# Danderson123/Amira

Hardware: AMD Instinct MI355X
Metric: gene-mers/s to corrected GeneMerGraph (higher is better)
Workload: dtype int32; 1 GPU; synthetic 1M reads x 60 genes, k=5, 20k-gene vocab: build + error-correction sweep (build, filter(3,1), correct, build, clip(5), correct, build); reads_per_gpu=1000000, genes_per_read=60, k=5, vocab=20000, gene_mers_per_gpu=56000000, final_nodes=472478, final_edges=1054844, multi_gpu=n/a

## Files before the change

### amira_amd/csrc/amg_api.hip

```cpp
#include <cstdarg>

#include "amg_device.h"

thread_local std::string g_amg_err;

int amg_fail(int code, const char* fmt, ...) {
  char buf[1024];
  va_list ap;
  va_start(ap, fmt);
  vsnprintf(buf, sizeof(buf), fmt, ap);
  va_end(ap);
  g_amg_err = buf;
  return code;
}

extern "C" const char* amg_last_error(void) { return g_amg_err.c_str(); }

void stages_reset(amg_ctx* c) {
  for (auto& s : c->stages) {
    (void)hipEventDestroy(s.a);
    (void)hipEventDestroy(s.b);
  }
  c->stages.clear();
}
// ... 122 lines not shown
  if (device < 0 || device >= n) return amg_fail(AMG_E_ARG, "device %d out of range [0,%d)", device, n);
  HIPCHK(hipSetDevice(device));
  amg_ctx* c = new amg_ctx();
  c->device = device;
  e = hipStreamCreateWithFlags(&c->stream, hipStreamNonBlocking);
  if (e != hipSuccess) {
    delete c;
    return amg_fail(AMG_E_HIP, "hipStreamCreate: %s", hipGetErrorString(e));
  }
  int r = c->status.ensure(ST_WORDS * sizeof(unsigned long long));
  if (r != AMG_OK) {
    delete c;
    return r;
  }
  const char* t = getenv("AMG_TIMING");
  c->timing = !(t && t[0] == '0');
  *out = c;
  return AMG_OK;
}

extern "C" int amg_destroy(amg_ctx* c) {
  if (!c) return AMG_OK;
  (void)hipSetDevice(c->device);
  (void)hipStreamSynchronize(c->stream);
  stages_reset(c);
  dist_release(c);
  bubbles_release(c);
  sketch_release(c);
  pop_release(c);
  DevBuf* all[] = {&c->tokens,    &c->read_off,  &c->gene_start, &c->gene_end,  &c->read_len,
                   &c->node_tab,  &c->edge_tab,  &c->tok_slot,   &c->tok_node,  &c->tok_dir, &c->tok_pair,
                   &c->node_tokens, &c->node_cov, &c->node_first, &c->node_comp, &c->node_alive,
                   &c->edge_src,  &c->edge_tgt,  &c->edge_sdir,  &c->edge_tdir, &c->edge_cov,
                   &c->edge_alive, &c->adj_off,  &c->adj_edge,   &c->read_fix, &c->ladj, &c->ladj_rows, &c->ladj_pos, &c->ladj_keys, &c->hub_bits, &c->pair_key, &c->pair_first, &c->pair_cnt, &c->match_read, &c->match_pos, &c->match_off, &c->match_wave,  &c->c_tokens_buf,
                   &c->c_read_off, &c->c_orig,   &c->c_changed,  &c->c_gstart,  &c->c_gend,
                   &c->c_read_len, &c->status,   &c->sort_tmp, &c->scan_state,   &c->s0, &c->s1, &c->s2, &c->s3,
                   &c->s4, &c->s5, &c->cnt_state, &c->cnt_list, &c->bnd_bits, &c->nw_rec, &c->gap_rec, &c->gm_mask, &c->gm_tab, &c->gm_res, &c->gm_list, &c->gm_q, &c->gm_pool, &c->gm_gene, &c->gm_fail, &c->gm_ctr, &c->routes_dev, &c->nw_big, &c->x_first, &c->x_slot, &c->x_final, &c->x_efirst, &c->x_eslot, &c->x_ecnt, &c->x_ncnt, &c->x_ftag, &c->f_ctrs, &c->x_first_all, &c->pos_off, &c->c_pos_off, &c->pos1_s, &c->pos1_e,
                   &c->c_src, &c->rd_src, &c->alt_tok_node, &c->alt_tok_dir, &c->alt_ntok, &c->alt_ncov, &c->alt_nfirst,
                   &c->alt_nalive, &c->alt_pkey, &c->alt_pfirst, &c->alt_pcnt};
  for (DevBuf* b : all) b->release();
  if (c->mail_host) (void)hipHostFree(c->mail_host);
  (void)hipStreamDestroy(c->stream);
  delete c;
  return AMG_OK;
}

extern "C" int amg_sync(amg_ctx* c) {
  if (!c) return amg_fail(AMG_E_ARG, "null ctx");
  HIPCHK(hipStreamSynchronize(c->stream));
  return AMG_OK;
}

extern "C" void* amg_stream(amg_ctx* c) { return c ? (void*)c->stream : nullptr; }

static int copy_in(amg_ctx* c, DevBuf& dst, const void* src, size_t bytes, int on_device) {
  if (on_device == 2) {
    dst.borrow(src, bytes);
    return AMG_OK;
  }
  AMGCHK(dst.ensure(bytes + 64));
  if (bytes)
    HIPCHK(hipMemcpyAsync(dst.p, src, bytes, on_device ? hipMemcpyDeviceToDevice : hipMemcpyHostToDevice,
                          c->stream));
  return AMG_OK;
}

extern "C" int amg_set_reads(amg_ctx* c, const int32_t* tokens, const int64_t* read_offsets,
// ... 322 lines not shown
```

### amira_amd/csrc/amg_correct.h

```cpp
#pragma once
#include "amg_device.h"

enum { RC_SKIP = 0, RC_COPY = 1, RC_DROP = 2, RC_TRIM = 3, RC_GAPPED = 4, RC_KEEP_ORIG = 5 };

struct CorrArgs {
  const int* tokens;
  const long long* read_off;
  const int* tok_node;
  const signed char* tok_dir;
  const unsigned char* read_fix;
  const long long* p0s;
  const long long* p0e;
  const long long* p1s;
  const long long* p1e;
  long long n0;
  const long long* pos_off;
  const long long* read_len;
  long long n_reads;
  int k, flip, have_pos;
  unsigned int* gflag;
  unsigned long long* max_bound;
  unsigned long long* lmask;
  unsigned long long* n_runs;
  unsigned char* cls;
  unsigned char* cls_final;
  int* r_start;
  int* r_end;
  unsigned int* bound;
  const long long* tmp_off;
  unsigned int* new_len;
  int* tmp_tok;
};

__device__ __forceinline__ void pos_base(const CorrArgs& a, long long off, const long long*& gs, const long long*& ge) {
  if (off < a.n0) {
    gs = a.p0s + off;
    ge = a.p0e + off;
  } else {
    gs = a.p1s + (off - a.n0);
    ge = a.p1e + (off - a.n0);
  }
}

// ... 136 lines not shown
  long long* o_off;
  int* o_orig;
  unsigned char* o_changed;
  long long* o_src;
  const long long* pos_new;
  long long* o_posoff;
  long long* o_rl;
  long long out_reads, out_tokens;
  unsigned long long* dead_kept;
};

struct CorrSwitches {
  bool gap_memo;
  bool gap_dfs_wave;
  bool fast_gapped;
  bool lean_gapped;
  int fast_nw;
  int nw_shortcuts;
  const char* node_bound;
  bool routes;
  const char* gap_pool;
  const char* memo_spill;
};

struct CorrScratch {
  size_t per_read = 0;
  unsigned char *cls = nullptr, *final_cls = nullptr;
  int *r_start = nullptr, *r_end = nullptr;
  long long *nw_size = nullptr, *nw_off = nullptr;
  unsigned int *bound = nullptr, *new_len = nullptr, *flag = nullptr;
  long long *tmp_off = nullptr, *new_idx = nullptr, *new_off = nullptr;
  int* tmp_tok = nullptr;
  long long *plen = nullptr, *poffs = nullptr, *pos_new = nullptr;
  unsigned long long *max_bound = nullptr, *n_general = nullptr;
  unsigned long long* n_runs = nullptr;
  unsigned long long* dead_kept = nullptr;
  bool count_alive = false;
  DevBuf* glist = nullptr;
  DevBuf* cand = nullptr;
  DevBuf* pool = nullptr;
  DevBuf* need_slow = nullptr;
};

struct CorrCounts {
  long long tmp_total = 0, n_gapped = 0, total_runs = 0;
  unsigned long long max_bound = 0;
  bool carry = false;
  long long out_reads = 0, out_tokens = 0, big_total = 0, pos_total = 0;
  unsigned long long n_general = 0;
  long long n_queries = 0;
  int pool_retries = 0;
  bool lean_ran = false, fast_ran = false, memo = false;
};

static void fill_pos_args(amg_ctx* c, CorrArgs& a) {
  a.p0s = c->have_pos ? c->gene_start.as<long long>() : nullptr;
  a.p0e = c->have_pos ? c->gene_end.as<long long>() : nullptr;
  a.p1s = c->pos1_s.as<long long>();
  a.p1e = c->pos1_e.as<long long>();
  a.n0 = c->pos_n0;
  a.pos_off = (c->have_pos && !c->pos_identity) ? c->pos_off.as<long long>() : nullptr;
}

int corr_gapped(amg_ctx* c, const CorrSwitches& sw, const CorrScratch& S, const CorrArgs& a, CorrCounts& n);
int corr_nw_sizes(amg_ctx* c, const CorrSwitches& sw, const CorrScratch& S, const CorrArgs& a, long long n_gapped,
                  FetchList& shape);
int corr_grow_pos_pools(amg_ctx* c, const CorrCounts& n);
int corr_positions(amg_ctx* c, const CorrSwitches& sw, const CorrScratch& S, const CorrArgs& a, const CorrCounts& n,
// ... 17 lines not shown
```

### amira_amd/csrc/amg_correct.hip

```cpp
#include "amg_correct.h"

__global__ __launch_bounds__(256) void k_count_alive(const unsigned char* __restrict__ alive, long long n,
                                                     unsigned long long* out) {
  __shared__ unsigned int s_part[4];
  unsigned int c = 0;
  for (long long i = ((long long)blockIdx.x * blockDim.x + threadIdx.x) * 4; i < n; i += (long long)gridDim.x * blockDim.x * 4) {
    if (i + 4 <= n) {
      const unsigned int w = *reinterpret_cast<const unsigned int*>(alive + i);
      c += __popc(w & 0x01010101u);
    } else {
      for (long long j = i; j < n; ++j) c += alive[j] ? 1u : 0u;
    }
  }
  for (int d = 32; d > 0; d >>= 1) c += (unsigned int)__shfl_xor((int)c, d, 64);
  if ((threadIdx.x & 63) == 0) s_part[threadIdx.x >> 6] = c;
  __syncthreads();
  if (threadIdx.x == 0 && (s_part[0] | s_part[1] | s_part[2] | s_part[3]))
    atomicAdd(out, (unsigned long long)s_part[0] + s_part[1] + s_part[2] + s_part[3]);
}

__global__ __launch_bounds__(256) void k_corr_classify(CorrArgs a) {
  const long long rbase = ((long long)blockIdx.x * 4 + (threadIdx.x >> 6)) * CLS_READS;
  if (rbase >= a.n_reads) return;
  const int lane = threadIdx.x & 63;
  const long long r = rbase + lane;
  const bool have = r < a.n_reads;
  const long long t0 = have ? a.read_off[r] : 0;
  const long long n = have ? (a.read_off[r + 1] - t0) - a.k + 1 : 0;
  const bool look = have && n > 0 && a.read_fix[r] != 0;
  unsigned long long lv = 0;
  unsigned long long todo = __ballot(look && n <= 64);
  while (todo) {
    int who[4];
    long long tj[4];
    int nj[4], v[4];
#pragma unroll
    for (int q = 0; q < 4; ++q) {
      who[q] = todo ? __ffsll((long long)todo) - 1 : -1;
      if (todo) todo &= todo - 1ull;
      tj[q] = who[q] >= 0 ? bcast_i64(t0, who[q]) : 0;
      nj[q] = who[q] >= 0 ? __builtin_amdgcn_readlane((int)n, who[q]) : 0;
    }
#pragma unroll
    for (int q = 0; q < 4; ++q) v[q] = lane < nj[q] ? a.tok_node[tj[q] + lane] : -1;
#pragma unroll
    for (int q = 0; q < 4; ++q) {
      const unsigned long long m = __ballot(v[q] >= 0);
      if (lane == who[q]) lv = m;
    }
  }
  long long first = n, last = -1;
  unsigned int runs = 0, live = 0;
  if (look && n <= 64) {
    first = lv ? (long long)__ffsll((long long)lv) - 1 : n;
    last = lv ? 63 - (long long)__clzll((long long)lv) : -1;
    live = (unsigned int)__popcll(lv);
    const unsigned long long inside =
        lv ? ((last == 63 ? ~0ull : ((1ull << (last + 1)) - 1ull)) & ~((1ull << first) - 1ull)) : 0ull;
    runs = (unsigned int)__popcll(~lv & inside & (lv >> 1));
  }
  unsigned long long big = __ballot(look && n > 64);
  while (big) {
    const int w = __ffsll((long long)big) - 1;
    big &= big - 1ull;
// ... 32 lines not shown
  unsigned char cls;
  int start = 0, end = -1;
  unsigned int bound = 0;
  unsigned int len_out = 0;
  if (n <= 0) {
    cls = RC_SKIP;
  } else if (!look) {
    cls = RC_COPY;
    len_out = (unsigned int)L;
  } else if (last < 0) {
    cls = RC_DROP;
  } else {
    start = (int)first;
    end = (int)last;
    if (runs == 0) {
      cls = RC_TRIM;
      len_out = (unsigned int)(end - start + a.k);
    } else {
      cls = RC_GAPPED;
      const unsigned int b1 = live + runs * (unsigned int)(2 * a.k) + (unsigned int)a.k;
      bound = b1 > (unsigned int)L ? b1 : (unsigned int)L;
    }
  }
  if (have) {
    a.cls[r] = cls;
    a.cls_final[r] = cls;
    a.r_start[r] = start;
    a.r_end[r] = end;
    a.bound[r] = bound;
    a.new_len[r] = len_out;
    a.gflag[r] = cls == RC_GAPPED ? 1u : 0u;
    a.lmask[r] = (cls == RC_GAPPED && n <= 64) ? lv : 0ull;
  }
  unsigned int mb = (have && cls == RC_GAPPED) ? bound : 0u;
  unsigned int nr = (have && cls == RC_GAPPED) ? runs : 0u;
  for (int d = 32; d > 0; d >>= 1) {
    const unsigned int o = (unsigned int)__shfl_xor((int)mb, d, 64);
    mb = mb > o ? mb : o;
    nr += (unsigned int)__shfl_xor((int)nr, d, 64);
  }
  if (lane == 0 && (unsigned long long)mb > *a.max_bound) atomicMax(a.max_bound, (unsigned long long)mb);
  if (lane == 0 && nr) atomicAdd(a.n_runs + 16 * (blockIdx.x & 15), (unsigned long long)nr);
}

__global__ __launch_bounds__(256) void k_corr_pack(PackArgs A) {
  const CorrArgs& a = A.a;
  const int lane = threadIdx.x & 63;
  const long long r = ((long long)blockIdx.x * 4 + (threadIdx.x >> 6)) * PACK_READS + lane;
  if (blockIdx.x == 0 && threadIdx.x == 0) A.o_off[A.out_reads] = A.out_tokens;
  long long dst = 0, src = 0;
  int n = 0;
  unsigned int dead = 0;
  if (r < a.n_reads && a.new_len[r] > 0) {
    dst = A.new_off[r];
    n = (int)a.new_len[r];
    const unsigned char fc = A.final_cls[r];
    if (fc == RC_KEEP_ORIG) {
      const long long nw = a.read_off[r + 1] - a.read_off[r] - a.k + 1;
      dead = nw <= 64 ? (unsigned int)(nw - __popcll(a.lmask[r])) : (unsigned int)nw;
    }
    long long poff = 0;
    if (fc == RC_GAPPED) {
      src = a.tmp_off[r] | (1ll << 62);
      if (a.have_pos) poff = A.pos_new[r];
    } else {
      const long long cut = fc == RC_TRIM ? a.r_start[r] : 0;
      src = a.read_off[r] + cut;
      if (a.have_pos) poff = (a.pos_off ? a.pos_off[r] : a.read_off[r]) + cut;
    }
    const long long q = A.new_idx[r];
    A.o_off[q] = dst;
    A.o_orig[q] = (int)r;
    A.o_changed[q] = (fc == RC_TRIM || fc == RC_GAPPED) ? 1 : 0;
    A.o_src[q] = fc == RC_GAPPED ? -1ll : src;
    if (a.have_pos) A.o_posoff[q] = poff;
// ... 38 lines not shown
  sw.gap_dfs_wave = is_one("AMG_GAP_DFS_WAVE");
  sw.fast_gapped = !is_one("AMG_NO_FAST_GAPPED");
  sw.lean_gapped = !is_one("AMG_NO_LEAN_GAPPED");
  sw.fast_nw = !is_one("AMG_NO_FAST_NW");
  sw.nw_shortcuts = !is_one("AMG_NW_NO_SHORTCUT");
  sw.node_bound = getenv("AMG_TEST_NODE_BOUND");
  sw.routes = is_one("AMG_CORR_ROUTES");
  sw.gap_pool = getenv("AMG_TEST_GAP_POOL");
  sw.memo_spill = getenv("AMG_TEST_MEMO_SPILL");
  return sw;
}

static int plan_per_read(amg_ctx* c, CorrScratch& S) {
  const size_t per_read = (size_t)(c->n_reads + 2);
  AMGCHK(c->s0.ensure(per_read * (1 + 1) + 64));
  AMGCHK(c->s1.ensure(per_read * sizeof(int) * 2 + per_read * sizeof(long long) * 2 + 64));
  AMGCHK(c->s2.ensure(per_read * sizeof(unsigned int) * 3));
  AMGCHK(c->s3.ensure(per_read * sizeof(long long) * 3));
  AMGCHK(c->gm_mask.ensure(per_read * sizeof(unsigned long long)));
  AMGCHK(c->gm_ctr.ensure((16 + 256 + 256 + 16) * sizeof(unsigned long long)));
  S.per_read = per_read;
  S.cls = c->s0.as<unsigned char>();
  S.final_cls = S.cls + per_read;
  S.r_start = c->s1.as<int>();
  S.r_end = S.r_start + per_read;
  S.nw_size = reinterpret_cast<long long*>(((uintptr_t)(S.r_end + per_read) + 15) & ~(uintptr_t)15);
  S.nw_off = S.nw_size + per_read;
  S.bound = c->s2.as<unsigned int>();
  S.new_len = S.bound + per_read;
  S.flag = S.new_len + per_read;
  S.tmp_off = c->s3.as<long long>();
  S.new_idx = S.tmp_off + per_read;
  S.new_off = S.new_idx + per_read;
  S.max_bound = S.n_general = c->status.as<unsigned long long>() + ST_MISC;
  S.n_runs = c->gm_ctr.as<unsigned long long>() + 16;
  S.dead_kept = S.n_runs + 256;
  S.count_alive = c->n_nodes >= (1ll << 20);
  S.glist = &c->c_orig;
  S.cand = &c->c_gstart;
  S.pool = &c->c_gend;
  S.need_slow = &c->c_changed;
  return AMG_OK;
}

static int plan_staging(amg_ctx* c, CorrScratch& S, long long tmp_total) {
  AMGCHK(c->c_tokens_buf.ensure((size_t)(tmp_total + 4) * sizeof(int)));
  AMGCHK(c->s4.ensure((size_t)(tmp_total + 4) * sizeof(int)));
  S.tmp_tok = c->s4.as<int>();
  return AMG_OK;
}

static int plan_positions(amg_ctx* c, CorrScratch& S, long long n_gapped) {
  AMGCHK(c->s5.ensure((size_t)(2 * (n_gapped + 2) + c->n_reads + 2) * sizeof(long long)));
  S.plen = c->s5.as<long long>();
  S.poffs = S.plen + (n_gapped + 2);
  S.pos_new = S.poffs + (n_gapped + 2);
  return AMG_OK;
}

static void corr_args(amg_ctx* c, const CorrScratch& S, CorrArgs& a) {
  a.tokens = c->tokens.as<int>();
  a.read_off = c->read_off.as<long long>();
  a.tok_node = c->tok_node.as<int>();
  a.tok_dir = c->tok_dir.as<signed char>();
  a.read_fix = c->read_fix.as<unsigned char>();
  fill_pos_args(c, a);
  a.read_len = c->have_read_len ? c->read_len.as<long long>() : nullptr;
  a.n_reads = c->n_reads;
  a.k = c->k;
  a.flip = c->two_v - 1;
  a.have_pos = c->have_pos ? 1 : 0;
  a.gflag = S.flag;
  a.max_bound = S.max_bound;
  a.lmask = c->gm_mask.as<unsigned long long>();
  a.n_runs = S.n_runs;
  a.cls = S.cls;
  a.cls_final = S.final_cls;
  a.r_start = S.r_start;
  a.r_end = S.r_end;
  a.bound = S.bound;
  a.tmp_off = S.tmp_off;
  a.new_len = S.new_len;
  a.tmp_tok = S.tmp_tok;
}

static int corr_classify(amg_ctx* c, const CorrScratch& S, const CorrArgs& a, CorrCounts& n) {
  hipStream_t st = c->stream;
  const long long R = c->n_reads;
  {
    ClearList cl;
    cl.add(S.bound, S.per_read * sizeof(unsigned int) * 3);
    cl.add(S.max_bound, sizeof(unsigned long long));
    cl.add(S.n_runs, (256 + 256 + 16) * sizeof(unsigned long long));
    AMGCHK(clear_many(c, cl));
  }
  if (R > 0) hipLaunchKernelGGL(k_corr_classify, dim3(nblk(R, 4 * CLS_READS)), dim3(256), 0, st, a);
  if (S.count_alive)
    hipLaunchKernelGGL(k_count_alive, dim3(128), dim3(256), 0, st, c->node_alive.as<unsigned char>(), c->n_nodes,
                       S.dead_kept + 256);
  AMGCHK(prim_exscan_u32_pair(c, S.bound, S.tmp_off, S.flag, S.new_idx, (size_t)R));
  FetchList l;
  l.add(S.tmp_off + R);
  l.add(S.max_bound);
  l.add(S.new_idx + R);
  for (int i = 0; i < 16; ++i) l.add(S.n_runs + 16 * i);
  unsigned long long v[3 + 16];
  AMGCHK(fetch(c, l, v));
  n.tmp_total = (long long)v[0];
  n.max_bound = v[1];
  n.n_gapped = (long long)v[2];
  for (int i = 0; i < 16; ++i) n.total_runs += (long long)v[3 + i];
  n.carry = n.n_gapped > 0 && c->have_pos;
  return AMG_OK;
}

static int corr_shape(amg_ctx* c, const CorrSwitches& sw, CorrScratch& S, const CorrArgs& a, CorrCounts& n) {
  const long long R = c->n_reads;
  AMGCHK(prim_exscan_keep_and_len(c, S.new_len, S.new_idx, S.new_off, (size_t)R));
  FetchList shape;
  shape.add(S.new_idx + R);
  shape.add(S.new_off + R);
  if (n.carry) {
    AMGCHK(plan_positions(c, S, n.n_gapped));
    AMGCHK(corr_nw_sizes(c, sw, S, a, n.n_gapped, shape));
  }
  unsigned long long v[5] = {0, 0, 0, 0, 0};
  AMGCHK(fetch(c, shape, v));
  n.out_reads = (long long)v[0];
  n.out_tokens = (long long)v[1];
  n.big_total = (long long)v[2];
  n.pos_total = (long long)v[3];
  n.n_general = v[4];
  return AMG_OK;
}

static int ensure_outputs(amg_ctx* c, const CorrCounts& n) {
  AMGCHK(c->c_tokens_buf.ensure((size_t)(n.out_tokens + 64) * sizeof(int)));
  AMGCHK(c->c_read_off.ensure((size_t)(n.out_reads + 2) * sizeof(long long)));
  AMGCHK(c->c_orig.ensure((size_t)(n.out_reads + 2) * sizeof(int)));
  AMGCHK(c->c_changed.ensure((size_t)(n.out_reads + 2)));
  AMGCHK(c->c_src.ensure((size_t)(n.out_reads + 2) * sizeof(long long)));
  if (c->have_pos) AMGCHK(c->c_pos_off.ensure((size_t)(n.out_reads + 2) * sizeof(long long)));
  if (c->have_read_len) AMGCHK(c->c_read_len.ensure((size_t)(n.out_reads + 2) * sizeof(long long)));
  return AMG_OK;
// ... 97 lines not shown
```

### amira_amd/csrc/amg_filter.hip

```cpp
#include "amg_rows.h"

__global__ void k_filter_nodes(const unsigned int* __restrict__ cov, unsigned char* __restrict__ alive,
                               long long n, unsigned int min_cov) {
  long long i = (long long)blockIdx.x * blockDim.x + threadIdx.x;
  if (i < n && alive[i] && cov[i] < min_cov) alive[i] = 0;
}

__device__ __forceinline__ void filter_edge(const int* __restrict__ src, const int* __restrict__ tgt,
                                            const unsigned int* __restrict__ cov,
                                            const unsigned char* __restrict__ node_alive,
                                            unsigned char* __restrict__ alive, long long e, unsigned int min_cov) {
  if (!alive[e]) return;
  if ((min_cov > 1 && cov[e] < min_cov) || !node_alive[src[e]] || !node_alive[tgt[e]]) alive[e] = 0;
}

__global__ __launch_bounds__(256) void k_filter_edges(const int* __restrict__ src, const int* __restrict__ tgt,
                                                      const unsigned int* __restrict__ cov,
                                                      const unsigned char* __restrict__ node_alive,
                                                      unsigned char* __restrict__ alive, long long n, unsigned int min_cov) {
  const long long q = (long long)blockIdx.x * blockDim.x + threadIdx.x;
  const long long e0 = 4 * q;
  if (e0 >= n) return;
  if (e0 + 4 > n) {
    for (long long e = e0; e < n; ++e) filter_edge(src, tgt, cov, node_alive, alive, e, min_cov);
    return;
  }
  const unsigned int a = reinterpret_cast<const unsigned int*>(alive)[q];
  if (a == 0u) return;
  const int4 s = reinterpret_cast<const int4*>(src)[q];
  const int4 t = reinterpret_cast<const int4*>(tgt)[q];
  uint4 c = make_uint4(min_cov, min_cov, min_cov, min_cov);
  if (min_cov > 1) c = reinterpret_cast<const uint4*>(cov)[q];
  const bool l0 = a & 0x000000ffu, l1 = a & 0x0000ff00u, l2 = a & 0x00ff0000u, l3 = a & 0xff000000u;
  const unsigned int ns0 = node_alive[l0 ? s.x : 0], ns1 = node_alive[l1 ? s.y : 0], ns2 = node_alive[l2 ? s.z : 0],
                     ns3 = node_alive[l3 ? s.w : 0];
  const unsigned int nt0 = node_alive[l0 ? t.x : 0], nt1 = node_alive[l1 ? t.y : 0], nt2 = node_alive[l2 ? t.z : 0],
                     nt3 = node_alive[l3 ? t.w : 0];
  unsigned int keep = 0u;
  if (ns0 && nt0 && c.x >= min_cov) keep |= 0x000000ffu;
  if (ns1 && nt1 && c.y >= min_cov) keep |= 0x0000ff00u;
  if (ns2 && nt2 && c.z >= min_cov) keep |= 0x00ff0000u;
  if (ns3 && nt3 && c.w >= min_cov) keep |= 0xff000000u;
  if ((a & keep) != a) reinterpret_cast<unsigned int*>(alive)[q] = a & keep;
}

#define READS_PER_WAVE 8
__global__ __launch_bounds__(256) void k_mask_reads(int* __restrict__ tok_node,
                                                    const long long* __restrict__ read_off,
                                                    long long n_reads,
                                                    const unsigned char* __restrict__ node_alive,
                                                    unsigned char* __restrict__ read_fix) {
  const long long rbase = ((long long)blockIdx.x * 4 + (threadIdx.x >> 6)) * READS_PER_WAVE;
  if (rbase >= n_reads) return;
  const int lane = threadIdx.x & 63;
  const long long off_l = (lane <= READS_PER_WAVE && rbase + lane <= n_reads) ? read_off[rbase + lane] : 0;
  long long a[READS_PER_WAVE], b[READS_PER_WAVE];
  int v[READS_PER_WAVE];
#pragma unroll
  for (int j = 0; j < READS_PER_WAVE; ++j) {
    a[j] = __shfl(off_l, j, 64);
    b[j] = rbase + j < n_reads ? __shfl(off_l, j + 1, 64) : a[j];
  }
#pragma unroll
  for (int j = 0; j < READS_PER_WAVE; ++j) v[j] = a[j] + lane < b[j] ? tok_node[a[j] + lane] : -1;
  bool dead[READS_PER_WAVE];
#pragma unroll
  for (int j = 0; j < READS_PER_WAVE; ++j) dead[j] = v[j] >= 0 && !node_alive[v[j]];
#pragma unroll
  for (int j = 0; j < READS_PER_WAVE; ++j) {
    if (dead[j]) tok_node[a[j] + lane] = -2;
    bool hit = dead[j];
    for (long long t = a[j] + 64 + lane; t < b[j]; t += 64) {
      const int n = tok_node[t];
      if (n >= 0 && !node_alive[n]) {
        tok_node[t] = -2;
        hit = true;
      }
    }
    if (__any(hit) && lane == 0) read_fix[rbase + j] = 1;
  }
}

static int apply_removals(amg_ctx* c, unsigned int min_edge_cov) {
  hipStream_t st = c->stream;
  if (min_edge_cov > 1) live_lists_after_edge_deaths(c);
  else live_lists_after_node_deaths(c);
  if (c->n_edges > 0)
    hipLaunchKernelGGL(k_filter_edges, dim3(nblk(c->n_edges, 4 * 256)), dim3(256), 0, st,
                       c->edge_src.as<int>(), c->edge_tgt.as<int>(), c->edge_cov.as<unsigned int>(),
                       c->node_alive.as<unsigned char>(), c->edge_alive.as<unsigned char>(),
                       c->n_edges, min_edge_cov);
  if (c->n_reads > 0)
    hipLaunchKernelGGL(k_mask_reads, dim3(nblk(c->n_reads, 4 * READS_PER_WAVE)), dim3(256), 0, st,
                       c->tok_node.as<int>(), c->read_off.as<long long>(), c->n_reads,
                       c->node_alive.as<unsigned char>(), c->read_fix.as<unsigned char>());
  return AMG_OK;
}

extern "C" int amg_filter(amg_ctx* c, uint32_t min_node_cov, uint32_t min_edge_cov) {
  NEED_BUILT(c);
  ctx_removal_begins(c);
  stages_reset(c);
  stage_begin(c, "filter");
  if (c->n_nodes > 0)
    hipLaunchKernelGGL(k_filter_nodes, dim3(nblk(c->n_nodes, 256)), dim3(256), 0, c->stream,
                       c->node_cov.as<unsigned int>(), c->node_alive.as<unsigned char>(),
                       c->n_nodes, min_node_cov);
  AMGCHK(apply_removals(c, min_edge_cov));
  stage_end(c);
  return AMG_OK;
}

__global__ void k_kill_listed(const int* __restrict__ ids, long long n, long long n_nodes,
                              unsigned char* __restrict__ alive) {
  long long i = (long long)blockIdx.x * blockDim.x + threadIdx.x;
  if (i >= n) return;
  int v = ids[i];
  if (v >= 0 && v < n_nodes) alive[v] = 0;
}

extern "C" int amg_remove_nodes(amg_ctx* c, const int32_t* node_ids, int64_t n) {
  NEED_BUILT(c);
  if (n < 0 || (n > 0 && !node_ids)) return amg_fail(AMG_E_ARG, "bad node list");
  if (n == 0) return AMG_OK;
  ctx_removal_begins(c);
  AMGCHK(c->s0.ensure((size_t)n * sizeof(int)));
  HIPCHK(hipMemcpyAsync(c->s0.p, node_ids, (size_t)n * sizeof(int), hipMemcpyHostToDevice, c->stream));
  hipLaunchKernelGGL(k_kill_listed, dim3(nblk(n, 256)), dim3(256), 0, c->stream, c->s0.as<int>(),
                     (long long)n, c->n_nodes, c->node_alive.as<unsigned char>());
  AMGCHK(apply_removals(c, 0));
  HIPCHK(hipStreamSynchronize(c->stream));
  return AMG_OK;
}

extern "C" int amg_remove_edges(amg_ctx* c, const int32_t* edge_ids, int64_t n) {
  NEED_BUILT(c);
  if (n < 0 || (n > 0 && !edge_ids)) return amg_fail(AMG_E_ARG, "bad edge list");
  if (n == 0) return AMG_OK;
// ... 284 lines not shown
```

### amira_amd/csrc/amg_internal.h

```cpp
#pragma once
#include <cstdint>
#include <cstdio>
#include <cstring>
#include <string>
#include <vector>

#include <hip/hip_runtime.h>

#include "amg_host.h"

#define HIPCHK(call)                                                                   \
  do {                                                                                 \
    hipError_t e_ = (call);                                                            \
    if (e_ != hipSuccess)                                                              \
      return amg_fail(AMG_E_HIP, "%s:%d %s -> %s", __FILE__, __LINE__, #call,          \
                      hipGetErrorString(e_));                                          \
  } while (0)
#define AMGCHK(call)                 \
  do {                               \
    int r_ = (call);                 \
    if (r_ != AMG_OK) return r_;     \
  } while (0)

struct DevBuf {
// ... 80 lines not shown
static const uint64_t kAmgSeed0 = 0x9E3779B97F4A7C15ull;
static const unsigned int kProbeLimit = 1024;

struct BuildSwitches {
  bool head_tiles_set = false;
  long long head_tiles = 0;
  int claim_shards = -1;
  bool tight_bits = false;
  bool key_fp = false;
  bool node_buckets = true;
  bool generic_k = false;
  int edge_lone = -1;
  bool edge_home = true;
  bool no_derive = false;
  int weak_fp = 0;
  bool count_inline = false;
  int count_list_seg = 1 << 30;
  bool count_debug = false;
};
BuildSwitches read_build_switches();

enum Overflow { OV_NONE = 0, OV_NODE_TABLE = 1, OV_EDGE_TABLE = 2, OV_COLLISION = 3 };
static inline int overflowed(Overflow* which, Overflow cause) { return *which = cause, AMG_E_OVERFLOW; }

struct DistState;
struct BubbleState;
struct SketchState;
struct PopState;

enum class LiveLists {
  Absent,
  Current,
  BehindNodes,
};

struct FpKeyList {
  const unsigned long long* first = nullptr;
  const unsigned int* slot = nullptr;
  unsigned long long* first_sorted = nullptr;
  unsigned int* slot_sorted = nullptr;
  long long n = 0;
};

struct amg_ctx {
  int device = 0;
  hipStream_t stream = nullptr;

  DevBuf tokens;
  DevBuf read_off;
  DevBuf gene_start;
  DevBuf gene_end;
  DevBuf read_len;
  bool have_pos = false, have_read_len = false;
  DevBuf pos_off, c_pos_off;
  DevBuf pos1_s, pos1_e;
  bool pos_identity = true;
  int64_t pos_n0 = 0, pos1_used = 0, c_pos1_used = 0;
  int64_t n_reads = 0, n_tokens = 0;
  int32_t two_v = 0;

  bool built = false;
  int32_t k = 0;
  uint64_t seed = kAmgSeed0;
  int64_t n_windows = 0, n_short = 0;
  int64_t n_nodes = 0, n_pairs = 0, n_edges = 0, n_components = 0;
  int64_t node_slots = 0, edge_slots = 0, retries = 0;
// ... 8 lines not shown
  int64_t tok_total = 0;

  DevBuf node_tab;
  DevBuf edge_tab;
  DevBuf tok_slot;
  DevBuf tok_node;
  DevBuf tok_dir;
  DevBuf tok_pair;
  bool packed_nodes = false;
  int weak_fp_builds = 0;
  bool dist_mode = false;
  bool count_inline = false;
  DevBuf node_tokens;
  DevBuf node_cov;
  DevBuf node_first;
  DevBuf node_comp;
  DevBuf node_alive;
  DevBuf edge_src, edge_tgt;
  DevBuf edge_sdir, edge_tdir;
  DevBuf edge_cov;
  DevBuf edge_alive;
  DevBuf pair_key, pair_first;
  DevBuf pair_cnt;
  DevBuf adj_off;
  DevBuf adj_edge;
  DevBuf ladj;
  DevBuf ladj_rows;
  DevBuf ladj_pos, ladj_keys;
  DevBuf hub_bits;
  LiveLists live_lists = LiveLists::Absent;
  bool comp_valid = false, adj_valid = false;
  bool pristine = false;
  DevBuf read_fix;

  bool have_corrected = false;
  bool pos0_own = false;
  int64_t c_reads = 0, c_tokens = 0;
  DevBuf c_tokens_buf, c_read_off, c_orig, c_changed, c_gstart, c_gend, c_read_len;

  DevBuf c_src, rd_src;
  bool c_derivable = false;
  bool derive_ready = false;
  bool derived = false;
  bool dist_candidate = false;
  bool edge_own_deaths = false;
  DevBuf alt_tok_node, alt_tok_dir, alt_ntok, alt_ncov, alt_nfirst, alt_nalive, alt_pkey, alt_pfirst, alt_pcnt;

  bool exact_keys = false;
  int x_bits = 0;
  bool x_fp = false;
  bool x_two = false;
  int x_kbits = 0;
  int64_t x_nspace = 0, x_espace = 0;
  bool dist_x = false;
  DevBuf x_first, x_slot;
  DevBuf x_final;
  DevBuf x_efirst, x_eslot;
  DevBuf x_ecnt;
  DevBuf x_ncnt;
  DevBuf x_ftag;
  DevBuf f_ctrs;
  DevBuf x_first_all;
  bool comp_from_claims = false;

  int world = 1;
  uint32_t dist_min_node = 1, dist_min_edge = 1;
// ... 218 lines not shown
```

### amira_amd/csrc/amg_state.h

```cpp
#pragma once
#include <cstdlib>

#include "amg_internal.h"

static inline int64_t ctx_hint_floor(int64_t n) { return n > 256 ? n : 256; }

static inline void ctx_reads_replaced(amg_ctx* c, int64_t n_reads, int64_t n_tokens, int32_t two_v) {
  c->n_reads = n_reads, c->n_tokens = n_tokens, c->two_v = two_v;
  c->have_pos = c->have_read_len = false;
  c->built = c->have_corrected = c->match_valid = false;
  c->derive_ready = c->dist_candidate = false;
  c->node_hint = c->hint_bound = 0;
  c->cnt_hint_reset = true;
}

static inline void ctx_positions_replaced(amg_ctx* c, int64_t n_tokens, bool own) {
  c->have_pos = c->pos_identity = true;
  c->pos0_own = own;
  c->pos_n0 = n_tokens;
  c->pos1_used = c->c_pos1_used = 0;
  c->have_corrected = c->have_read_len = false;
}
static inline void ctx_read_lengths_set(amg_ctx* c) { c->have_read_len = true; }

static inline void ctx_corrected_begun(amg_ctx* c) { c->have_corrected = c->c_derivable = false; }
static inline void ctx_corrected_made(amg_ctx* c, int64_t reads, int64_t tokens, int64_t pos1_used, bool only_drops_and_trims,
                                      int64_t bound, const char* test_bound) {
  c->c_reads = reads, c->c_tokens = tokens;
  c->c_pos1_used = pos1_used;
  c->c_derivable = only_drops_and_trims && !c->edge_own_deaths;
  c->c_node_bound = test_bound ? atoll(test_bound) : bound;
  c->c_node_bound_k = c->k;
  c->have_corrected = true;
}

static inline void ctx_corrected_adopted(amg_ctx* c, bool compacted) {
  c->derive_ready = c->c_derivable;
  c->dist_candidate = c->dist_mode;
  if (c->have_pos && compacted) {
    c->pos0_own = c->pos_identity = true;
    c->pos_n0 = c->c_tokens;
    c->pos1_used = c->c_pos1_used = 0;
  } else if (c->have_pos) {
    c->pos_identity = false;
    c->pos1_used = c->c_pos1_used;
  }
  c->n_reads = c->c_reads, c->n_tokens = c->c_tokens;
  c->c_derivable = c->have_corrected = c->built = c->match_valid = false;
  if (c->c_node_bound > 0 && c->c_node_bound_k == c->k && (c->node_hint == 0 || c->c_node_bound < c->node_hint))
    c->node_hint = ctx_hint_floor(c->c_node_bound);
  c->c_node_bound = 0;
}

static inline bool ctx_take_derive_offer(amg_ctx* c) {
  const bool offered = c->derive_ready;
  c->derive_ready = c->dist_candidate = false;
  return offered;
}
static inline bool ctx_build_begins(amg_ctx* c) {
  c->derived = c->built = c->have_corrected = c->match_valid = false;
  c->retries = c->tok_base = 0;
  c->tok_total = c->n_tokens;
  return ctx_take_derive_offer(c);
}
static inline void ctx_build_from_reads(amg_ctx* c, int32_t k, bool merged) {
  c->k = k;
  c->dist_mode = merged;
  c->comp_from_claims = false;
  if (!merged && c->hint_bound > 0) {
    if (c->hint_bound_k == k) c->node_hint = ctx_hint_floor(c->hint_bound);
    c->hint_bound = 0;
  }
}

static inline void ctx_graph_in_place(amg_ctx* c, int64_t seen, bool derived) {
  c->live_lists = LiveLists::Absent;
  c->pristine = !c->comp_from_claims;
  c->edge_own_deaths = c->comp_valid = c->adj_valid = false;
  c->n_components = 0;
  c->built = true;
  c->derived = derived;
  c->node_hint = ctx_hint_floor(seen);
}

static inline void ctx_removal_begins(amg_ctx* c) { c->have_corrected = false; }
static inline void live_lists_after_node_deaths(amg_ctx* c) {
  if (c->live_lists == LiveLists::Current)
    c->live_lists = getenv("AMG_NO_LADJ_PATCH") ? LiveLists::Absent : LiveLists::BehindNodes;
  c->pristine = c->match_valid = false;
}
static inline void live_lists_after_edge_deaths(amg_ctx* c) {
  c->live_lists = LiveLists::Absent;
  c->edge_own_deaths = true;
  c->pristine = c->match_valid = false;
}
static inline void live_lists_made(amg_ctx* c) { c->live_lists = LiveLists::Current; }
static inline void ctx_match_begun(amg_ctx* c) { c->match_valid = false; }
```

Measured before the change: 10.72 billion gene-mers/s.

## Cache per-read alive-window masks from filtering and reuse them in correction classify

The read-masking kernel now records, for each read, a 64-bit ballot of which windows still map to live nodes, and tracks the validity of these masks in context state. The correction classify kernel uses them instead of re-gathering tok_node and node_alive per window. The change also vectorises the node filter and alive-count kernels, and replaces per-wave global atomics in classify with a block-level reduction into 16 striped slots. In exchange it adds an extra per-read buffer and state-invalidation logic that must stay correct, plus a unit test for those state transitions.

```diff
diff --git a/amira_amd/csrc/amg_api.hip b/amira_amd/csrc/amg_api.hip
--- a/amira_amd/csrc/amg_api.hip
+++ b/amira_amd/csrc/amg_api.hip
@@ -178,7 +178,7 @@
                    &c->node_tab,  &c->edge_tab,  &c->tok_slot,   &c->tok_node,  &c->tok_dir, &c->tok_pair,
                    &c->node_tokens, &c->node_cov, &c->node_first, &c->node_comp, &c->node_alive,
                    &c->edge_src,  &c->edge_tgt,  &c->edge_sdir,  &c->edge_tdir, &c->edge_cov,
-                   &c->edge_alive, &c->adj_off,  &c->adj_edge,   &c->read_fix, &c->ladj, &c->ladj_rows, &c->ladj_pos, &c->ladj_keys, &c->hub_bits, &c->pair_key, &c->pair_first, &c->pair_cnt, &c->match_read, &c->match_pos, &c->match_off, &c->match_wave,  &c->c_tokens_buf,
+                   &c->edge_alive, &c->adj_off,  &c->adj_edge,   &c->read_fix, &c->win_mask, &c->ladj, &c->ladj_rows, &c->ladj_pos, &c->ladj_keys, &c->hub_bits, &c->pair_key, &c->pair_first, &c->pair_cnt, &c->match_read, &c->match_pos, &c->match_off, &c->match_wave,  &c->c_tokens_buf,
                    &c->c_read_off, &c->c_orig,   &c->c_changed,  &c->c_gstart,  &c->c_gend,
                    &c->c_read_len, &c->status,   &c->sort_tmp, &c->scan_state,   &c->s0, &c->s1, &c->s2, &c->s3,
                    &c->s4, &c->s5, &c->cnt_state, &c->cnt_list, &c->bnd_bits, &c->nw_rec, &c->gap_rec, &c->gm_mask, &c->gm_tab, &c->gm_res, &c->gm_list, &c->gm_q, &c->gm_pool, &c->gm_gene, &c->gm_fail, &c->gm_ctr, &c->routes_dev, &c->nw_big, &c->x_first, &c->x_slot, &c->x_final, &c->x_efirst, &c->x_eslot, &c->x_ecnt, &c->x_ncnt, &c->x_ftag, &c->f_ctrs, &c->x_first_all, &c->pos_off, &c->c_pos_off, &c->pos1_s, &c->pos1_e,
diff --git a/amira_amd/csrc/amg_correct.h b/amira_amd/csrc/amg_correct.h
--- a/amira_amd/csrc/amg_correct.h
+++ b/amira_amd/csrc/amg_correct.h
@@ -9,6 +9,7 @@
   const int* tok_node;
   const signed char* tok_dir;
   const unsigned char* read_fix;
+  const unsigned long long* win_mask;
   const long long* p0s;
   const long long* p0e;
   const long long* p1s;
@@ -211,8 +212,9 @@
   long long *tmp_off = nullptr, *new_idx = nullptr, *new_off = nullptr;
   int* tmp_tok = nullptr;
   long long *plen = nullptr, *poffs = nullptr, *pos_new = nullptr;
-  unsigned long long *max_bound = nullptr, *n_general = nullptr;
+  unsigned long long* n_general = nullptr;
   unsigned long long* n_runs = nullptr;
+  unsigned long long* max_bound = nullptr;
   unsigned long long* dead_kept = nullptr;
   bool count_alive = false;
   DevBuf* glist = nullptr;
diff --git a/amira_amd/csrc/amg_correct.hip b/amira_amd/csrc/amg_correct.hip
--- a/amira_amd/csrc/amg_correct.hip
+++ b/amira_amd/csrc/amg_correct.hip
@@ -1,16 +1,16 @@
 #include "amg_correct.h"
 
+#define COUNT_PER 16
 __global__ __launch_bounds__(256) void k_count_alive(const unsigned char* __restrict__ alive, long long n,
                                                      unsigned long long* out) {
   __shared__ unsigned int s_part[4];
   unsigned int c = 0;
-  for (long long i = ((long long)blockIdx.x * blockDim.x + threadIdx.x) * 4; i < n; i += (long long)gridDim.x * blockDim.x * 4) {
-    if (i + 4 <= n) {
-      const unsigned int w = *reinterpret_cast<const unsigned int*>(alive + i);
-      c += __popc(w & 0x01010101u);
-    } else {
-      for (long long j = i; j < n; ++j) c += alive[j] ? 1u : 0u;
-    }
+  const long long i = ((long long)blockIdx.x * blockDim.x + threadIdx.x) * COUNT_PER;
+  if (i + COUNT_PER <= n) {
+    const uint4 w = *reinterpret_cast<const uint4*>(alive + i);
+    c = __popc(w.x & 0x01010101u) + __popc(w.y & 0x01010101u) + __popc(w.z & 0x01010101u) + __popc(w.w & 0x01010101u);
+  } else {
+    for (long long j = i; j < n; ++j) c += alive[j] ? 1u : 0u;
   }
   for (int d = 32; d > 0; d >>= 1) c += (unsigned int)__shfl_xor((int)c, d, 64);
   if ((threadIdx.x & 63) == 0) s_part[threadIdx.x >> 6] = c;
@@ -21,7 +21,6 @@
 
 __global__ __launch_bounds__(256) void k_corr_classify(CorrArgs a) {
   const long long rbase = ((long long)blockIdx.x * 4 + (threadIdx.x >> 6)) * CLS_READS;
-  if (rbase >= a.n_reads) return;
   const int lane = threadIdx.x & 63;
   const long long r = rbase + lane;
   const bool have = r < a.n_reads;
@@ -29,7 +28,8 @@
   const long long n = have ? (a.read_off[r + 1] - t0) - a.k + 1 : 0;
   const bool look = have && n > 0 && a.read_fix[r] != 0;
   unsigned long long lv = 0;
-  unsigned long long todo = __ballot(look && n <= 64);
+  if (a.win_mask && look && n <= 64) lv = a.win_mask[r] & (n == 64 ? ~0ull : (1ull << n) - 1ull);
+  unsigned long long todo = a.win_mask ? 0ull : __ballot(look && n <= 64);
   while (todo) {
     int who[4];
     long long tj[4];
@@ -128,6 +128,7 @@
     a.gflag[r] = cls == RC_GAPPED ? 1u : 0u;
     a.lmask[r] = (cls == RC_GAPPED && n <= 64) ? lv : 0ull;
   }
+  __shared__ unsigned int s_mb[4], s_nr[4];
   unsigned int mb = (have && cls == RC_GAPPED) ? bound : 0u;
   unsigned int nr = (have && cls == RC_GAPPED) ? runs : 0u;
   for (int d = 32; d > 0; d >>= 1) {
@@ -135,8 +136,17 @@
     mb = mb > o ? mb : o;
     nr += (unsigned int)__shfl_xor((int)nr, d, 64);
   }
-  if (lane == 0 && (unsigned long long)mb > *a.max_bound) atomicMax(a.max_bound, (unsigned long long)mb);
-  if (lane == 0 && nr) atomicAdd(a.n_runs + 16 * (blockIdx.x & 15), (unsigned long long)nr);
+  if (lane == 0) {
+    s_mb[threadIdx.x >> 6] = mb;
+    s_nr[threadIdx.x >> 6] = nr;
+  }
+  __syncthreads();
+  if (threadIdx.x == 0) {
+    const unsigned int m01 = s_mb[0] > s_mb[1] ? s_mb[0] : s_mb[1], m23 = s_mb[2] > s_mb[3] ? s_mb[2] : s_mb[3];
+    const unsigned int m = m01 > m23 ? m01 : m23, s = s_nr[0] + s_nr[1] + s_nr[2] + s_nr[3];
+    if (m) atomicMax(a.max_bound + 16 * (blockIdx.x & 15), (unsigned long long)m);
+    if (s) atomicAdd(a.n_runs + 16 * (blockIdx.x & 15), (unsigned long long)s);
+  }
 }
 
 __global__ __launch_bounds__(256) void k_corr_pack(PackArgs A) {
@@ -241,8 +251,9 @@
   S.tmp_off = c->s3.as<long long>();
   S.new_idx = S.tmp_off + per_read;
   S.new_off = S.new_idx + per_read;
-  S.max_bound = S.n_general = c->status.as<unsigned long long>() + ST_MISC;
+  S.n_general = c->status.as<unsigned long long>() + ST_MISC;
   S.n_runs = c->gm_ctr.as<unsigned long long>() + 16;
+  S.max_bound = S.n_runs + 8;
   S.dead_kept = S.n_runs + 256;
   S.count_alive = c->n_nodes >= (1ll << 20);
   S.glist = &c->c_orig;
@@ -273,6 +284,7 @@
   a.tok_node = c->tok_node.as<int>();
   a.tok_dir = c->tok_dir.as<signed char>();
   a.read_fix = c->read_fix.as<unsigned char>();
+  a.win_mask = c->win_masks == WindowMasks::Current ? c->win_mask.as<unsigned long long>() : nullptr;
   fill_pos_args(c, a);
   a.read_len = c->have_read_len ? c->read_len.as<long long>() : nullptr;
   a.n_reads = c->n_reads;
@@ -299,26 +311,25 @@
   {
     ClearList cl;
     cl.add(S.bound, S.per_read * sizeof(unsigned int) * 3);
-    cl.add(S.max_bound, sizeof(unsigned long long));
     cl.add(S.n_runs, (256 + 256 + 16) * sizeof(unsigned long long));
     AMGCHK(clear_many(c, cl));
   }
   if (R > 0) hipLaunchKernelGGL(k_corr_classify, dim3(nblk(R, 4 * CLS_READS)), dim3(256), 0, st, a);
   if (S.count_alive)
-    hipLaunchKernelGGL(k_count_alive, dim3(128), dim3(256), 0, st, c->node_alive.as<unsigned char>(), c->n_nodes,
+    hipLaunchKernelGGL(k_count_alive, dim3(nblk(c->n_nodes, 256 * COUNT_PER)), dim3(256), 0, st, c->node_alive.as<unsigned char>(), c->n_nodes,
                        S.dead_kept + 256);
   AMGCHK(prim_exscan_u32_pair(c, S.bound, S.tmp_off, S.flag, S.new_idx, (size_t)R));
   FetchList l;
   l.add(S.tmp_off + R);
-  l.add(S.max_bound);
   l.add(S.new_idx + R);
   for (int i = 0; i < 16; ++i) l.add(S.n_runs + 16 * i);
-  unsigned long long v[3 + 16];
+  for (int i = 0; i < 16; ++i) l.add(S.max_bound + 16 * i);
+  unsigned long long v[2 + 16 + 16];
   AMGCHK(fetch(c, l, v));
   n.tmp_total = (long long)v[0];
-  n.max_bound = v[1];
-  n.n_gapped = (long long)v[2];
-  for (int i = 0; i < 16; ++i) n.total_runs += (long long)v[3 + i];
+  n.n_gapped = (long long)v[1];
+  for (int i = 0; i < 16; ++i) n.total_runs += (long long)v[2 + i];
+  for (int i = 0; i < 16; ++i) n.max_bound = n.max_bound > v[18 + i] ? n.max_bound : v[18 + i];
   n.carry = n.n_gapped > 0 && c->have_pos;
   return AMG_OK;
 }
diff --git a/amira_amd/csrc/amg_filter.hip b/amira_amd/csrc/amg_filter.hip
--- a/amira_amd/csrc/amg_filter.hip
+++ b/amira_amd/csrc/amg_filter.hip
@@ -1,9 +1,24 @@
 #include "amg_rows.h"
 
-__global__ void k_filter_nodes(const unsigned int* __restrict__ cov, unsigned char* __restrict__ alive,
-                               long long n, unsigned int min_cov) {
-  long long i = (long long)blockIdx.x * blockDim.x + threadIdx.x;
-  if (i < n && alive[i] && cov[i] < min_cov) alive[i] = 0;
+__global__ __launch_bounds__(256) void k_filter_nodes(const unsigned int* __restrict__ cov, unsigned char* __restrict__ alive,
+                                                      long long n, unsigned int min_cov) {
+  const long long q = (long long)blockIdx.x * blockDim.x + threadIdx.x;
+  const long long i0 = 4 * q;
+  if (i0 >= n) return;
+  if (i0 + 4 > n) {
+    for (long long i = i0; i < n; ++i)
+      if (alive[i] && cov[i] < min_cov) alive[i] = 0;
+    return;
+  }
+  const unsigned int a = reinterpret_cast<const unsigned int*>(alive)[q];
+  if (a == 0u) return;
+  const uint4 c = reinterpret_cast<const uint4*>(cov)[q];
+  unsigned int keep = 0u;
+  if (c.x >= min_cov) keep |= 0x000000ffu;
+  if (c.y >= min_cov) keep |= 0x0000ff00u;
+  if (c.z >= min_cov) keep |= 0x00ff0000u;
+  if (c.w >= min_cov) keep |= 0xff000000u;
+  if ((a & keep) != a) reinterpret_cast<unsigned int*>(alive)[q] = a & keep;
 }
 
 __device__ __forceinline__ void filter_edge(const int* __restrict__ src, const int* __restrict__ tgt,
@@ -49,7 +64,8 @@
                                                     const long long* __restrict__ read_off,
                                                     long long n_reads,
                                                     const unsigned char* __restrict__ node_alive,
-                                                    unsigned char* __restrict__ read_fix) {
+                                                    unsigned char* __restrict__ read_fix,
+                                                    unsigned long long* __restrict__ win_mask) {
   const long long rbase = ((long long)blockIdx.x * 4 + (threadIdx.x >> 6)) * READS_PER_WAVE;
   if (rbase >= n_reads) return;
   const int lane = threadIdx.x & 63;
@@ -66,6 +82,13 @@
   bool dead[READS_PER_WAVE];
 #pragma unroll
   for (int j = 0; j < READS_PER_WAVE; ++j) dead[j] = v[j] >= 0 && !node_alive[v[j]];
+  unsigned long long mine = 0;
+#pragma unroll
+  for (int j = 0; j < READS_PER_WAVE; ++j) {
+    const unsigned long long m = __ballot(v[j] >= 0 && !dead[j]);
+    if (lane == j) mine = m;
+  }
+  if (lane < READS_PER_WAVE && rbase + lane < n_reads) win_mask[rbase + lane] = mine;
 #pragma unroll
   for (int j = 0; j < READS_PER_WAVE; ++j) {
     if (dead[j]) tok_node[a[j] + lane] = -2;
@@ -90,10 +113,13 @@
                        c->edge_src.as<int>(), c->edge_tgt.as<int>(), c->edge_cov.as<unsigned int>(),
                        c->node_alive.as<unsigned char>(), c->edge_alive.as<unsigned char>(),
                        c->n_edges, min_edge_cov);
+  AMGCHK(c->win_mask.ensure((size_t)(c->n_reads + 2) * sizeof(unsigned long long)));
   if (c->n_reads > 0)
     hipLaunchKernelGGL(k_mask_reads, dim3(nblk(c->n_reads, 4 * READS_PER_WAVE)), dim3(256), 0, st,
                        c->tok_node.as<int>(), c->read_off.as<long long>(), c->n_reads,
-                       c->node_alive.as<unsigned char>(), c->read_fix.as<unsigned char>());
+                       c->node_alive.as<unsigned char>(), c->read_fix.as<unsigned char>(),
+                       c->win_mask.as<unsigned long long>());
+  window_masks_made(c);
   return AMG_OK;
 }
 
@@ -103,7 +129,7 @@
   stages_reset(c);
   stage_begin(c, "filter");
   if (c->n_nodes > 0)
-    hipLaunchKernelGGL(k_filter_nodes, dim3(nblk(c->n_nodes, 256)), dim3(256), 0, c->stream,
+    hipLaunchKernelGGL(k_filter_nodes, dim3(nblk(c->n_nodes, 4 * 256)), dim3(256), 0, c->stream,
                        c->node_cov.as<unsigned int>(), c->node_alive.as<unsigned char>(),
                        c->n_nodes, min_node_cov);
   AMGCHK(apply_removals(c, min_edge_cov));
diff --git a/amira_amd/csrc/amg_internal.h b/amira_amd/csrc/amg_internal.h
--- a/amira_amd/csrc/amg_internal.h
+++ b/amira_amd/csrc/amg_internal.h
@@ -136,6 +136,11 @@
   Absent,
   Current,
   BehindNodes,
+};
+
+enum class WindowMasks {
+  Absent,
+  Current,
 };
 
 struct FpKeyList {
@@ -210,6 +215,8 @@
   bool comp_valid = false, adj_valid = false;
   bool pristine = false;
   DevBuf read_fix;
+  DevBuf win_mask;
+  WindowMasks win_masks = WindowMasks::Absent;
 
   bool have_corrected = false;
   bool pos0_own = false;
diff --git a/amira_amd/csrc/amg_state.h b/amira_amd/csrc/amg_state.h
--- a/amira_amd/csrc/amg_state.h
+++ b/amira_amd/csrc/amg_state.h
@@ -4,6 +4,9 @@
 #include "amg_internal.h"
 
 static inline int64_t ctx_hint_floor(int64_t n) { return n > 256 ? n : 256; }
+
+static inline void window_masks_made(amg_ctx* c) { c->win_masks = WindowMasks::Current; }
+static inline void window_masks_void(amg_ctx* c) { c->win_masks = WindowMasks::Absent; }
 
 static inline void ctx_reads_replaced(amg_ctx* c, int64_t n_reads, int64_t n_tokens, int32_t two_v) {
   c->n_reads = n_reads, c->n_tokens = n_tokens, c->two_v = two_v;
@@ -12,6 +15,7 @@
   c->derive_ready = c->dist_candidate = false;
   c->node_hint = c->hint_bound = 0;
   c->cnt_hint_reset = true;
+  window_masks_void(c);
 }
 
 static inline void ctx_positions_replaced(amg_ctx* c, int64_t n_tokens, bool own) {
@@ -47,6 +51,7 @@
   }
   c->n_reads = c->c_reads, c->n_tokens = c->c_tokens;
   c->c_derivable = c->have_corrected = c->built = c->match_valid = false;
+  window_masks_void(c);
   if (c->c_node_bound > 0 && c->c_node_bound_k == c->k && (c->node_hint == 0 || c->c_node_bound < c->node_hint))
     c->node_hint = ctx_hint_floor(c->c_node_bound);
   c->c_node_bound = 0;
@@ -61,6 +66,7 @@
   c->derived = c->built = c->have_corrected = c->match_valid = false;
   c->retries = c->tok_base = 0;
   c->tok_total = c->n_tokens;
+  window_masks_void(c);
   return ctx_take_derive_offer(c);
 }
 static inline void ctx_build_from_reads(amg_ctx* c, int32_t k, bool merged) {
@@ -75,6 +81,7 @@
 
 static inline void ctx_graph_in_place(amg_ctx* c, int64_t seen, bool derived) {
   c->live_lists = LiveLists::Absent;
+  window_masks_void(c);
   c->pristine = !c->comp_from_claims;
   c->edge_own_deaths = c->comp_valid = c->adj_valid = false;
   c->n_components = 0;
diff --git a/amira_amd/csrc/window_masks_check.cpp b/amira_amd/csrc/window_masks_check.cpp
--- /dev/null
+++ b/amira_amd/csrc/window_masks_check.cpp
@@ -0,0 +1,114 @@
+#include <cstdio>
+#include <cstdlib>
+
+#include "amg_state.h"
+
+#define CHECK(cond)                                                                          \
+  do {                                                                                       \
+    if (!(cond)) {                                                                           \
+      fprintf(stderr, "window_masks_check: line %d: %s does not hold\n", __LINE__, #cond);  \
+      exit(1);                                                                               \
+    }                                                                                        \
+  } while (0)
+
+enum Event {
+  READS_REPLACED, POSITIONS_CALLERS, POSITIONS_OWN, LENGTHS_SET, CORRECTED_BEGUN, MADE_TRIMS_ONLY, MADE_OTHER, ADOPTED,
+  ADOPTED_COMPACTED, OFFER_TAKEN, BUILD_BEGINS, FROM_READS_SINGLE, FROM_READS_MERGED, GRAPH_IN_PLACE, GRAPH_DERIVED,
+  REMOVAL_BEGINS, NODES_DIED, EDGE_DIED, LISTS_MADE, MATCH_BEGUN, MASKS_MADE, MASKS_VOID, N_EVENTS
+};
+static void apply(amg_ctx* c, int e) {
+  switch (e) {
+    case READS_REPLACED: ctx_reads_replaced(c, 7, 70, 20); break;
+    case POSITIONS_CALLERS: ctx_positions_replaced(c, 70, false); break;
+    case POSITIONS_OWN: ctx_positions_replaced(c, 70, true); break;
+    case LENGTHS_SET: ctx_read_lengths_set(c); break;
+    case CORRECTED_BEGUN: ctx_corrected_begun(c); break;
+    case MADE_TRIMS_ONLY: ctx_corrected_made(c, 5, 50, 0, true, 300, nullptr); break;
+    case MADE_OTHER: ctx_corrected_made(c, 5, 50, 0, false, 300, nullptr); break;
+    case ADOPTED: ctx_corrected_adopted(c, false); break;
+    case ADOPTED_COMPACTED: ctx_corrected_adopted(c, true); break;
+    case OFFER_TAKEN: (void)ctx_take_derive_offer(c); break;
+    case BUILD_BEGINS: (void)ctx_build_begins(c); break;
+    case FROM_READS_SINGLE: ctx_build_from_reads(c, 3, false); break;
+    case FROM_READS_MERGED: ctx_build_from_reads(c, 3, true); break;
+    case GRAPH_IN_PLACE: ctx_graph_in_place(c, 1000, false); break;
+    case GRAPH_DERIVED: ctx_graph_in_place(c, 1000, true); break;
+    case REMOVAL_BEGINS: ctx_removal_begins(c); break;
+    case NODES_DIED: live_lists_after_node_deaths(c); break;
+    case EDGE_DIED: live_lists_after_edge_deaths(c); break;
+    case LISTS_MADE: live_lists_made(c); break;
+    case MATCH_BEGUN: ctx_match_begun(c); break;
+    case MASKS_MADE: window_masks_made(c); break;
+    case MASKS_VOID: window_masks_void(c); break;
+  }
+}
+static WindowMasks expected(int e, WindowMasks was) {
+  switch (e) {
+    case MASKS_MADE: return WindowMasks::Current;
+    case READS_REPLACED: case ADOPTED: case ADOPTED_COMPACTED: case BUILD_BEGINS: case GRAPH_IN_PLACE: case GRAPH_DERIVED:
+    case MASKS_VOID:
+      return WindowMasks::Absent;
+    default: return was;
+  }
+}
+
+int main() {
+  long long n = 0;
+  for (int e = 0; e < N_EVENTS; ++e)
+    for (int had_pos = 0; had_pos < 2; ++had_pos)
+      for (WindowMasks was : {WindowMasks::Absent, WindowMasks::Current}) {
+        amg_ctx c;
+        c.have_pos = had_pos != 0;
+        c.win_masks = was;
+        apply(&c, e);
+        CHECK(c.win_masks == expected(e, was));
+        ++n;
+      }
+  {
+    amg_ctx c;
+    CHECK(c.win_masks == WindowMasks::Absent);
+    ctx_reads_replaced(&c, 7, 70, 20);
+    (void)ctx_build_begins(&c);
+    ctx_build_from_reads(&c, 3, false);
+    ctx_graph_in_place(&c, 100, false);
+    CHECK(c.win_masks == WindowMasks::Absent);
+    ctx_removal_begins(&c);
+    live_lists_after_node_deaths(&c);
+    CHECK(c.win_masks == WindowMasks::Absent);
+    window_masks_made(&c);
+    CHECK(c.win_masks == WindowMasks::Current);
+    ctx_removal_begins(&c);
+    live_lists_after_node_deaths(&c);
+    window_masks_made(&c);
+    ctx_removal_begins(&c);
+    live_lists_after_edge_deaths(&c);
+    CHECK(c.win_masks == WindowMasks::Current);
+    ctx_corrected_begun(&c);
+    ctx_corrected_made(&c, 5, 50, 0, true, 90, nullptr);
+    CHECK(c.win_masks == WindowMasks::Current);
+    ctx_corrected_adopted(&c, false);
+    CHECK(c.win_masks == WindowMasks::Absent);
+    window_masks_made(&c);
+    (void)ctx_build_begins(&c);
+    CHECK(c.win_masks == WindowMasks::Absent);
+    window_masks_made(&c);
+    ctx_graph_in_place(&c, 90, true);
+    CHECK(c.win_masks == WindowMasks::Absent);
+    (void)ctx_build_begins(&c);
+    ctx_build_from_reads(&c, 3, false);
+    ctx_graph_in_place(&c, 100, false);
+    ctx_corrected_begun(&c);
+    CHECK(c.win_masks == WindowMasks::Absent);
+    window_masks_made(&c);
+    (void)ctx_build_begins(&c);
+    ctx_build_from_reads(&c, 3, true);
+    CHECK(c.win_masks == WindowMasks::Absent);
+    ctx_graph_in_place(&c, 100, false);
+    CHECK(c.win_masks == WindowMasks::Absent);
+    window_masks_made(&c);
+    ctx_reads_replaced(&c, 3, 30, 20);
+    CHECK(c.win_masks == WindowMasks::Absent);
+  }
+  printf("window_masks_check: %lld transitions and the sequences passed\n", n);
+  return 0;
+}
```

Measured after the change: 10.94 billion gene-mers/s (median of 6 runs). 1.02x the previous value.
